# vsergeev/luaradio

Measured on NVIDIA H100. Metric: WBFM-mono chain Msamples/s (input samples) @N H100; FIR-128 HBM GB/s vs roofline, higher is better.
Workload: dtype f32

## Files before the change

### luaradio_b200/csrc/tuner.cu

```cuda
#include "common.cuh"
#include "blocks.h"

#include <cmath>
#include <cstdlib>
#include <cstring>
#include <new>
#include <string>
#include <type_traits>
#include <vector>

namespace lrb {

namespace {

#ifndef LRB_PT_THREADS
#define LRB_PT_THREADS 64
#define LRB_PT_R 8
#define LRB_PT_CTAS 8
#define LRB_PT_PREFETCH 9
#define LRB_PT_BATCH 7
#endif
#ifndef LRB_PT_CTAS_BULK
#define LRB_PT_CTAS_BULK 5
#endif
#ifndef LRB_PT_EXPERIMENT
#define LRB_PT_EXPERIMENT 0
#endif
#ifndef LRB_PT_EARLY_REST
#define LRB_PT_EARLY_REST 0
#endif
constexpr int PT_THREADS = LRB_PT_THREADS;
constexpr int PT_R = LRB_PT_R;
constexpr int PT_TO = PT_THREADS * PT_R;
constexpr int PT_MAXTAPS = 144;
constexpr int PT_BATCH = LRB_PT_BATCH;

constexpr int PT_MAXIT = 48;
struct PolyParams {
    float hr[PT_MAXTAPS];
    float hs[PT_MAXTAPS / 2];
    float2 step[PT_MAXIT];
    uint64_t turns_fix;
    uint64_t g0;
    long long off;
    int M;
    float pole_c;
    float pole_cp[6];
};
constexpr int PT_POLE_WARM = (64 % LRB_PT_R == 0) ? 64 : ((72 % LRB_PT_R == 0) ? 72 : 4 * LRB_PT_R);
static_assert(PT_POLE_WARM % LRB_PT_R == 0 && PT_POLE_WARM % 4 == 0 && PT_POLE_WARM >= 64, "pole warm-up must cover whole threads");

template <int D, int Q>
struct PolyShape {
    static constexpr int RD = PT_R * D;
    static constexpr int T = Q * D + 1;
    static constexpr int SPAN = (PT_TO + Q - 1) * D + 1;
    static constexpr int PAIRS = (SPAN + 1) / 2;
    static constexpr int ITERS = (PAIRS + PT_THREADS - 1) / PT_THREADS;
    static constexpr int LOADED = 2 * ITERS * PT_THREADS;
    __host__ __device__ static constexpr int pad(int e) { return e + 2 * (e / RD); }
    static constexpr int ELEMS = LOADED + 2 * (LOADED / RD) + 2;
    static constexpr size_t SMEM = (size_t)ELEMS * sizeof(float2);
    static constexpr int RAW = ELEMS;
    static constexpr size_t SMEM_BULK = (size_t)(ELEMS + LOADED) * sizeof(float2);
    static constexpr int NSEG = (LOADED + RD - 1) / RD;
    static constexpr int PPS = RD / 2;
    static constexpr int RG = PT_THREADS / PPS;
    static constexpr int RITERS = (NSEG + RG - 1) / RG;
};

__device__ __forceinline__ uint32_t smem_addr(const void* p) { return (uint32_t)__cvta_generic_to_shared(p); }
__device__ __forceinline__ void mbar_init(uint64_t* bar) {
    asm volatile("mbarrier.init.shared::cta.b64 [%0], 1;\n\tfence.mbarrier_init.release.cluster;\n\t"
                 "fence.proxy.async.shared::cta;" :: "r"(smem_addr(bar)) : "memory");
}
__device__ __forceinline__ void mbar_expect_tx(uint64_t* bar, uint32_t bytes) {
    asm volatile("mbarrier.arrive.expect_tx.shared::cta.b64 _, [%0], %1;" :: "r"(smem_addr(bar)), "r"(bytes) : "memory");
}
__device__ __forceinline__ void mbar_wait(uint64_t* bar, uint32_t parity) {
    asm volatile("{\n\t.reg .pred p;\n\tLRB_WAIT_%=:\n\t"
                 "mbarrier.try_wait.parity.shared::cta.b64 p, [%0], %1;\n\t"
                 "@!p bra LRB_WAIT_%=;\n\t}" :: "r"(smem_addr(bar)), "r"(parity) : "memory");
}
__device__ __forceinline__ void fence_proxy_async() { asm volatile("fence.proxy.async.shared::cta;" ::: "memory"); }
__device__ __forceinline__ void bulk_g2s(void* dst, const void* src, uint32_t bytes, uint64_t* bar) {
    asm volatile("cp.async.bulk.shared::cluster.global.mbarrier::complete_tx::bytes [%0], [%1], %2, [%3];"
                 :: "r"(smem_addr(dst)), "l"(src), "r"(bytes), "r"(smem_addr(bar)) : "memory");
}

template <int B, int E, typename F>
__device__ __forceinline__ void static_for(F&& f) {
    if constexpr (B < E) {
        f(std::integral_constant<int, B>{});
        static_for<B + 1, E>(f);
    }
}

constexpr int DISC_OV = 4;
constexpr int DISC_TAIL = 4;
template <bool DISC>
struct TileStride { static constexpr int TS = DISC ? PT_TO - DISC_OV - DISC_TAIL : PT_TO; };

template <int D, int Q, bool ROT, bool DISC, bool EDGE, bool REAL = false, bool POLE = false>
__global__ void __launch_bounds__(PT_THREADS, (!EDGE && !REAL && DISC) ? LRB_PT_CTAS_BULK : LRB_PT_CTAS)
polyphase_crcf_kernel(const float2* __restrict__ x, const float2* __restrict__ hist, long long n,
                      void* __restrict__ yv, long long n_out, const __grid_constant__ PolyParams P,
                      long long t_lo, long long t_hi,
                      const float2* __restrict__ prev_in, float2* __restrict__ prev_out, float inv_gain) {
    using S = PolyShape<D, Q>;
    static_assert(!(REAL && (ROT || DISC)), "the real-stream variant has no translator / discriminator");
    static_assert(REAL || !POLE, "the fused pole exists in the real-stream variant only");
    constexpr int PW = POLE ? PT_POLE_WARM : 0;
    constexpr int PAY = PT_TO - PW;
    constexpr int TS = REAL ? 2 * PAY : TileStride<DISC>::TS;
    constexpr int NPRE = S::ITERS < LRB_PT_PREFETCH ? S::ITERS : LRB_PT_PREFETCH;
    constexpr int LANE1 = PAY * D;
    const float* __restrict__ xr = reinterpret_cast<const float*>(x);
    const float* __restrict__ histr = reinterpret_cast<const float*>(hist);
    extern __shared__ __align__(16) float2 smem[];
    __shared__ float2 s_edge[PT_THREADS / 32];
    const int tid = threadIdx.x, lane = tid & 31, warp = tid >> 5;
    const int Hm1 = P.M - 1;

    constexpr bool BULK = !EDGE && !REAL && DISC;
    constexpr bool FFA = BULK && LRB_PT_EXPERIMENT != 2;
    __shared__ float2 s_ffa[FFA ? 4 : 1][PT_THREADS / 32];
    __shared__ __align__(8) uint64_t s_bar;
    uint32_t bar_phase = 0;

    float2 A0 = make_float2(1.f, 0.f), A1 = make_float2(1.f, 0.f);
    const int rg = tid / S::PPS, rw = tid - rg * S::PPS;
    constexpr int NE0 = (BULK && ROT) ? S::RITERS : 1;
    float2 E0[NE0];
    float2 W1 = make_float2(1.f, 0.f);
    if constexpr (BULK && ROT) {
        W1 = phasor_from_fix(P.turns_fix);
#pragma unroll
        for (int it = 0; it < NE0; ++it)
            E0[it] = phasor_from_fix(P.turns_fix * (uint64_t)((rg + S::RG * it) * S::RD + 2 * rw));
    } else if constexpr (ROT) {
        A0 = phasor_from_fix(P.turns_fix * (uint64_t)(2 * tid));
        A1 = phasor_from_fix(P.turns_fix * (uint64_t)(2 * tid + 1));
    }
    const bool rot_last = rg < S::RG && (rg + S::RG * (S::RITERS - 1)) * S::RD + 2 * rw < S::LOADED;
    auto tile_of = [&](long long idx) -> long long { return EDGE ? (idx < t_lo ? idx : t_hi + (idx - t_lo)) : (t_lo + idx); };
    const long long n_work = EDGE ? 0 : (t_hi - t_lo);
    long long widx = blockIdx.x;

    auto issue_tile = [&](long long idx) {
        if (tid == 0) {
            fence_proxy_async();
            mbar_expect_tx(&s_bar, (uint32_t)(S::LOADED * sizeof(float2)));
            bulk_g2s(smem + S::RAW, x + (P.off + tile_of(idx) * (long long)(TS * D)), (uint32_t)(S::LOADED * sizeof(float2)), &s_bar);
        }
    };
    if constexpr (BULK) {
        if (tid == 0) mbar_init(&s_bar);
        __syncthreads();
        if (widx < n_work) issue_tile(widx);
    }

    auto ld_pair = [&](long long Bt, int k) -> float4 {
        if constexpr (REAL) {
            const float2* pa = reinterpret_cast<const float2*>(xr + Bt) + (tid + k * PT_THREADS);
            const float2 a = __ldcs(pa), b = __ldcs(pa + LANE1 / 2);
            return make_float4(a.x, b.x, a.y, b.y);
        } else {
            return __ldcs(reinterpret_cast<const float4*>(x + Bt) + (tid + k * PT_THREADS));
        }
    };
    float4 pre[NPRE];
    constexpr int REST = (S::ITERS - NPRE) < PT_BATCH ? (S::ITERS - NPRE) : PT_BATCH;
    float4 rest[REST > 0 ? REST : 1];
    if constexpr (!EDGE && !BULK) {
        if (widx < n_work) {
            const long long Bt = P.off + tile_of(widx) * (long long)(TS * D);
#pragma unroll
            for (int k = 0; k < NPRE; ++k) pre[k] = ld_pair(Bt, k);
            if constexpr (LRB_PT_EARLY_REST) {
#pragma unroll
                for (int k = 0; k < REST; ++k) rest[k] = ld_pair(Bt, NPRE + k);
            }
        }
    }

    for (;;) {
        if constexpr (!EDGE) { if (widx >= n_work) break; }
        const long long tile = tile_of(widx);
        const long long B = P.off + tile * (long long)(TS * D);
        const long long m0 = tile * TS - (DISC ? DISC_OV : 0) - PW;

        auto stage_pair = [&](float4 v, int it) {
            const int u = tid + it * PT_THREADS;
            float2 a = make_float2(v.x, v.y), b = make_float2(v.z, v.w);
            if constexpr (ROT) {
                const float2 st = P.step[it];
                a = cmul(a, cmul(A0, st));
                b = cmul(b, cmul(A1, st));
            }
            *reinterpret_cast<float4*>(smem + S::pad(2 * u)) = make_float4(a.x, a.y, b.x, b.y);
        };
        if constexpr (BULK) {
            if (LRB_PT_EXPERIMENT != 1 || widx == blockIdx.x) {
                mbar_wait(&s_bar, bar_phase);
                bar_phase ^= 1;
                if (rg < S::RG) {
                    const float2* src = smem + S::RAW + rg * S::RD + 2 * rw;
                    float2* dst = smem + rg * (S::RD + 2) + 2 * rw;
#pragma unroll
                    for (int it = 0; it < S::RITERS; ++it) {
                        if (it == S::RITERS - 1 && !rot_last) break;
                        float4 v = *reinterpret_cast<const float4*>(src + it * S::RG * S::RD);
                        if constexpr (ROT) {
                            const float2 a = cmul(make_float2(v.x, v.y), E0[it]);
                            const float2 b = cmul(make_float2(v.z, v.w), cmul(E0[it], W1));
                            v = make_float4(a.x, a.y, b.x, b.y);
                        }
                        *reinterpret_cast<float4*>(dst + it * S::RG * (S::RD + 2)) = v;
                    }
                }
            }
        } else if constexpr (!EDGE && LRB_PT_EXPERIMENT == 1) {
            if (widx == blockIdx.x) {
#pragma unroll 1
                for (int it = 0; it < S::ITERS; ++it) stage_pair(ld_pair(B, it), it);
            }
        } else if constexpr (!EDGE) {
            if constexpr (!LRB_PT_EARLY_REST) {
#pragma unroll
                for (int k = 0; k < REST; ++k) rest[k] = ld_pair(B, NPRE + k);
            }
#pragma unroll
            for (int k = 0; k < NPRE; ++k) stage_pair(pre[k], k);
#pragma unroll
            for (int k = 0; k < REST; ++k) stage_pair(rest[k], NPRE + k);
#pragma unroll 1
            for (int it0 = NPRE + REST; it0 < S::ITERS; it0 += PT_BATCH) {
                float4 buf[PT_BATCH];
#pragma unroll
                for (int k = 0; k < PT_BATCH; ++k)
                    if (it0 + k < S::ITERS) buf[k] = ld_pair(B, it0 + k);
#pragma unroll
                for (int k = 0; k < PT_BATCH; ++k)
                    if (it0 + k < S::ITERS) stage_pair(buf[k], it0 + k);
            }
        } else {
#pragma unroll 7
            for (int it = 0; it < S::ITERS; ++it) {
                const long long i0 = B + 2LL * (tid + it * PT_THREADS);
                if constexpr (REAL) {
                    auto g = [&](long long i) -> float {
                        return (i >= 0) ? (i < n ? __ldg(xr + i) : 0.f) : ((Hm1 + i >= 0) ? __ldg(histr + (Hm1 + i)) : 0.f);
                    };
                    stage_pair(make_float4(g(i0), g(i0 + LANE1), g(i0 + 1), g(i0 + 1 + LANE1)), it);
                    continue;
                }
                const float2 a = (i0 >= 0) ? (i0 < n ? __ldg(x + i0) : make_float2(0.f, 0.f))
                                           : ((Hm1 + i0 >= 0) ? __ldg(hist + (Hm1 + i0)) : make_float2(0.f, 0.f));
                const long long i1 = i0 + 1;
                const float2 b = (i1 >= 0) ? (i1 < n ? __ldg(x + i1) : make_float2(0.f, 0.f))
                                           : ((Hm1 + i1 >= 0) ? __ldg(hist + (Hm1 + i1)) : make_float2(0.f, 0.f));
                stage_pair(make_float4(a.x, a.y, b.x, b.y), it);
            }
        }
        __syncthreads();

        if constexpr (BULK && LRB_PT_EXPERIMENT != 1) {
            if (widx + gridDim.x < n_work) issue_tile(widx + gridDim.x);
        }
        if constexpr (!EDGE && !BULK && LRB_PT_EXPERIMENT != 1) {
            const long long nidx = widx + gridDim.x;
            if (nidx < n_work) {
                const long long Bn = P.off + tile_of(nidx) * (long long)(TS * D);
#pragma unroll
                for (int k = 0; k < NPRE; ++k) pre[k] = ld_pair(Bn, k);
            }
        }

        float2 acc[PT_R];
#pragma unroll
        for (int r = 0; r < PT_R; ++r) acc[r] = make_float2(0.f, 0.f);
        const float2* tb = smem + tid * (S::RD + 2);
        auto load_block = [&](auto jc, float2 (&xs)[D]) {
            constexpr int j = decltype(jc)::value;
            constexpr int e0 = j * D;
            if constexpr (j == PT_R + Q - 1) {
                xs[0] = tb[S::pad(e0)];
            } else {
                static_for<0, D>([&](auto pc) {
                    constexpr int pp = decltype(pc)::value;
                    constexpr int e = e0 + pp;
                    if constexpr ((e & 1) && pp >= 1) {
                    } else if constexpr (!(e & 1) && pp + 1 < D) {
                        const float4 v = *reinterpret_cast<const float4*>(tb + S::pad(e));
                        xs[pp] = make_float2(v.x, v.y);
                        xs[pp + 1] = make_float2(v.z, v.w);
                    } else {
                        xs[pp] = tb[S::pad(e)];
                    }
                });
            }
        };
        float2 ffa_a0, ffa_fs, ffa_fb, ffa_sp;
        const float hq = P.hr[Q * D];
        if constexpr (FFA) {
            static_assert(Q % 2 == 0 && PT_R % 2 == 0 && (Q / 2) * D <= PT_MAXTAPS / 2, "fast-FIR split needs even Q and R");
            static_assert(DISC_TAIL >= 1, "the tile's last output has no A_{R/2}");
            constexpr int QH = Q / 2, KP = PT_R / 2;
            float2 fa[KP], fb[KP], fs[KP], uo[D], an;
#pragma unroll
            for (int k = 0; k < KP; ++k) fa[k] = fb[k] = fs[k] = make_float2(0.f, 0.f);
            static_for<0, PT_R + Q>([&](auto jc) {
                constexpr int j = decltype(jc)::value;
                float2 xs[D];
                load_block(jc, xs);
                if constexpr (j == PT_R + Q - 1) {
                } else if constexpr (j % 2 == 0) {
                    constexpr int i = j / 2;
                    static_for<0, KP>([&](auto kc) {
                        constexpr int k = decltype(kc)::value, q = i - k;
                        if constexpr (q >= 0 && q < QH) {
                            static_for<0, D>([&](auto pc) {
                                constexpr int pp = decltype(pc)::value;
                                const float h = P.hr[2 * q * D + pp];
                                fa[k] = ffma2(xs[pp], make_float2(h, h), fa[k]);
                            });
                        }
                    });
                    if constexpr (i >= 1 && i - 1 <= KP - 1 + QH - 1) {
                        float2 v[D];
#pragma unroll
                        for (int pp = 0; pp < D; ++pp) v[pp] = fadd2(uo[pp], xs[pp]);
                        static_for<0, KP>([&](auto kc) {
                            constexpr int k = decltype(kc)::value, q = i - 1 - k;
                            if constexpr (q >= 0 && q < QH) {
                                static_for<0, D>([&](auto pc) {
                                    constexpr int pp = decltype(pc)::value;
                                    const float h = P.hs[q * D + pp];
                                    fs[k] = ffma2(v[pp], make_float2(h, h), fs[k]);
                                });
                            }
                        });
                    }
                } else {
                    constexpr int i = (j - 1) / 2;
                    static_for<0, KP>([&](auto kc) {
                        constexpr int k = decltype(kc)::value, q = i - k;
                        if constexpr (q >= 0 && q < QH) {
                            static_for<0, D>([&](auto pc) {
                                constexpr int pp = decltype(pc)::value;
                                const float h = P.hr[(2 * q + 1) * D + pp];
                                fb[k] = ffma2(xs[pp], make_float2(h, h), fb[k]);
                            });
                        }
                    });
#pragma unroll
                    for (int pp = 0; pp < D; ++pp) uo[pp] = xs[pp];
                }
                if constexpr (j == 2 * QH - 1) {
                    an = make_float2(__shfl_down_sync(0xffffffffu, fa[0].x, 1), __shfl_down_sync(0xffffffffu, fa[0].y, 1));
                }
                if constexpr (j >= Q) {
                    constexpr int r = j - Q, k = r / 2;
                    if constexpr (r % 2 == 0) {
                        acc[r] = ffma2(xs[0], make_float2(hq, hq), fadd2(fa[k], fb[k]));
                    } else if constexpr (k + 1 < KP) {
                        acc[r] = ffma2(xs[0], make_float2(hq, hq), fsub2(fsub2(fs[k], fa[k + 1]), fb[k]));
                    } else {
                        acc[r] = ffma2(xs[0], make_float2(hq, hq), fsub2(fsub2(fs[k], an), fb[k]));
                        ffa_a0 = fa[0]; ffa_fs = fs[k]; ffa_fb = fb[k]; ffa_sp = xs[0];
                    }
                }
            });
        } else {
            static_for<0, (LRB_PT_EXPERIMENT == 2 ? 1 : PT_R + Q)>([&](auto jc) {
                constexpr int j = decltype(jc)::value;
                float2 xs[D];
                load_block(jc, xs);
                static_for<0, PT_R>([&](auto rc) {
                    constexpr int r = decltype(rc)::value;
                    constexpr int qq = j - r;
                    if constexpr (qq >= 0 && qq <= Q) {
                        static_for<0, D>([&](auto pc) {
                            constexpr int pp = decltype(pc)::value;
                            if constexpr (qq * D + pp < S::T) {
                                const float h = P.hr[qq * D + pp];
                                acc[r] = ffma2(xs[pp], make_float2(h, h), acc[r]);
                            }
                        });
                    }
                });
            });
        }
        if constexpr (!EDGE && !BULK && LRB_PT_EARLY_REST) {
            const long long nidx = widx + gridDim.x;
            if (nidx < n_work) {
                const long long Bn = P.off + tile_of(nidx) * (long long)(TS * D);
#pragma unroll
                for (int k = 0; k < REST; ++k) rest[k] = ld_pair(Bn, NPRE + k);
            }
        }
        if constexpr (ROT && !DISC) {
            const float2 Pt = phasor_from_fix(P.turns_fix * (P.g0 + (uint64_t)B));
#pragma unroll
            for (int r = 0; r < PT_R; ++r) acc[r] = cmul(acc[r], Pt);
        }

        const long long mbase = m0 + (long long)tid * PT_R;
        if constexpr (POLE) {
            const float c = P.pole_c;
            if (tile == 0 && tid < PW / PT_R) {
#pragma unroll
                for (int r = 0; r < PT_R; ++r) acc[r].x = 0.f;
                if (tid == PW / PT_R - 1) acc[PT_R - 1].x = __ldg(reinterpret_cast<const float*>(prev_in));
            }
#pragma unroll
            for (int r = 1; r < PT_R; ++r) acc[r] = ffma2(acc[r - 1], make_float2(c, c), acc[r]);
            float2 Bv = acc[PT_R - 1];
#pragma unroll
            for (int k = 0; k < 5; ++k) {
                const float2 o = make_float2(__shfl_up_sync(0xffffffffu, Bv.x, 1 << k), __shfl_up_sync(0xffffffffu, Bv.y, 1 << k));
                if (lane >= (1 << k)) Bv = ffma2(o, make_float2(P.pole_cp[k], P.pole_cp[k]), Bv);
            }
            if (lane == 31) s_edge[warp] = Bv;
            float2 prevB = make_float2(__shfl_up_sync(0xffffffffu, Bv.x, 1), __shfl_up_sync(0xffffffffu, Bv.y, 1));
            if (lane == 0) prevB = make_float2(0.f, 0.f);
            __syncthreads();
            float2 carryW = make_float2(0.f, 0.f);
            for (int w = 0; w < warp; ++w) carryW = ffma2(carryW, make_float2(P.pole_cp[5], P.pole_cp[5]), s_edge[w]);
            float f_lane = 1.f;
#pragma unroll
            for (int k = 0; k < 5; ++k) if (lane & (1 << k)) f_lane *= P.pole_cp[k];
            const float2 excl = ffma2(carryW, make_float2(f_lane, f_lane), prevB);
            float cpow = c;
#pragma unroll
            for (int r = 0; r < PT_R; ++r) { acc[r] = ffma2(excl, make_float2(cpow, cpow), acc[r]); cpow *= c; }
        }
        if constexpr (REAL) {
            float* y = reinterpret_cast<float*>(yv);
#pragma unroll
            for (int half = 0; half < 2; ++half) {
                const long long mb = mbase + half * PAY;
                if (POLE && tid < PW / PT_R) continue;
                float v[PT_R];
#pragma unroll
                for (int r = 0; r < PT_R; ++r) v[r] = half ? acc[r].y : acc[r].x;
                if (mb + PT_R <= n_out && ((reinterpret_cast<uintptr_t>(y + mb) & 15) == 0)) {
#pragma unroll
                    for (int r = 0; r < PT_R; r += 4)
                        __stcs(reinterpret_cast<float4*>(y + mb + r), make_float4(v[r], v[r + 1], v[r + 2], v[r + 3]));
                } else {
#pragma unroll
                    for (int r = 0; r < PT_R; ++r)
                        if (mb + r < n_out) y[mb + r] = v[r];
                }
                if constexpr (POLE) {
                    if (mb <= n_out - 1 && n_out - 1 < mb + PT_R) {
#pragma unroll
                        for (int r = 0; r < PT_R; ++r)
                            if (mb + r == n_out - 1) *reinterpret_cast<float*>(prev_out) = v[r];
                    }
                }
            }
            __syncthreads();
        } else if constexpr (!DISC) {
            float2* y = reinterpret_cast<float2*>(yv);
            if (mbase + PT_R <= n_out && ((reinterpret_cast<uintptr_t>(y + mbase) & 15) == 0)) {
                float4* y4 = reinterpret_cast<float4*>(y + mbase);
#pragma unroll
                for (int r = 0; r < PT_R; r += 2)
                    __stcs(y4 + r / 2, make_float4(acc[r].x, acc[r].y, acc[r + 1].x, acc[r + 1].y));
            } else {
#pragma unroll
                for (int r = 0; r < PT_R; ++r)
                    if (mbase + r < n_out) y[mbase + r] = acc[r];
            }
            __syncthreads();
        } else {
            float* yd = reinterpret_cast<float*>(yv);
            float2 left;
            left.x = __shfl_up_sync(0xffffffffu, acc[PT_R - 1].x, 1);
            left.y = __shfl_up_sync(0xffffffffu, acc[PT_R - 1].y, 1);
            if constexpr (FFA) {
                if (lane == 0) s_ffa[0][warp] = ffa_a0;
                if (lane == 31) { s_ffa[1][warp] = ffa_fs; s_ffa[2][warp] = ffa_fb; s_ffa[3][warp] = ffa_sp; }
            } else {
                if (lane == 31) s_edge[warp] = acc[PT_R - 1];
            }
            __syncthreads();
            if constexpr (FFA) {
                auto last_out = [&](int w, float2 a) {
                    return ffma2(s_ffa[3][w], make_float2(hq, hq), fsub2(fsub2(s_ffa[1][w], a), s_ffa[2][w]));
                };
                if (lane == 0 && warp > 0) left = last_out(warp - 1, ffa_a0);
                if (lane == 31 && warp + 1 < PT_THREADS / 32) acc[PT_R - 1] = last_out(warp, s_ffa[0][warp + 1]);
            } else {
                if (lane == 0 && warp > 0) left = s_edge[warp - 1];
            }
            bool zero_prev = false;
            if (EDGE && tid == 0 && tile == 0) {
                const float2 Pt = ROT ? phasor_from_fix(P.turns_fix * (P.g0 + (uint64_t)B)) : make_float2(1.f, 0.f);
                const float2 pv = __ldg(prev_in);
                acc[DISC_OV - 1] = cmul(pv, make_float2(Pt.x, -Pt.y));
                zero_prev = pv.x == 0.f && pv.y == 0.f;
            }
            const int s0 = tid * PT_R;
            float* yt = yd + m0;
            float dout[PT_R];
#pragma unroll
            for (int r = 0; r < PT_R; r += 2) {
                const float2 c0 = acc[r], p0 = (r == 0) ? left : acc[r - 1];
                const float2 c1 = acc[r + 1], p1 = acc[r];
                const float2 t0 = ffma2(c0, make_float2(p0.x, p0.x), fmul2(make_float2(c0.y, -c0.x), make_float2(p0.y, p0.y)));
                const float2 t1 = ffma2(c1, make_float2(p1.x, p1.x), fmul2(make_float2(c1.y, -c1.x), make_float2(p1.y, p1.y)));
                const float2 ang = fast_atan2f_x2(make_float2(t0.y, t1.y), make_float2(t0.x, t1.x));
                dout[r] = ang.x * inv_gain;
                dout[r + 1] = ang.y * inv_gain;
            }
            if (EDGE && zero_prev) {
                const float2 Pt = ROT ? phasor_from_fix(P.turns_fix * (P.g0 + (uint64_t)B)) : make_float2(1.f, 0.f);
                const float2 ya = ROT ? cmul(acc[DISC_OV], Pt) : acc[DISC_OV];
                const float pz = 0.f, nz = -0.f;
                const float re = __fsub_rn(__fmul_rn(ya.x, pz), __fmul_rn(ya.y, nz));
                const float im = __fadd_rn(__fmul_rn(ya.x, nz), __fmul_rn(ya.y, pz));
                dout[DISC_OV] = atan2f(im, re) * inv_gain;
            }
            if constexpr (!EDGE) {
                if (((reinterpret_cast<uintptr_t>(yt) + DISC_OV * sizeof(float)) & 15) == 0) {
                    static_assert(DISC_OV == 4 && DISC_TAIL == 4 && PT_R % 4 == 0,
                                  "thread 0 skips exactly its first float4, the last thread exactly its last");
#pragma unroll
                    for (int r = 0; r < PT_R; r += 4)
                        if ((tid > 0 || r >= DISC_OV) && (tid < PT_THREADS - 1 || r < PT_R - DISC_TAIL))
                            *reinterpret_cast<float4*>(yt + s0 + r) = make_float4(dout[r], dout[r + 1], dout[r + 2], dout[r + 3]);
                } else {
#pragma unroll
                    for (int r = 0; r < PT_R; ++r)
                        if (s0 + r >= DISC_OV && s0 + r < PT_TO - DISC_TAIL) yt[s0 + r] = dout[r];
                }
            } else {
                const long long room = n_out - m0;
                const int lim = room < (long long)(PT_TO - DISC_TAIL) ? (int)room : PT_TO - DISC_TAIL;
#pragma unroll
                for (int r = 0; r < PT_R; ++r) {
                    const int sl = s0 + r;
                    if (sl >= DISC_OV && sl < lim) {
                        yt[sl] = dout[r];
                        if ((long long)sl == room - 1) {
                            const float2 Pt = ROT ? phasor_from_fix(P.turns_fix * (P.g0 + (uint64_t)B)) : make_float2(1.f, 0.f);
                            *prev_out = cmul(acc[r], Pt);
                        }
                    }
                }
            }
        }
        if constexpr (EDGE) break;
        widx += gridDim.x;
    }
}

template <int D, int Q, bool ROT, bool DISC, bool REAL = false, bool POLE = false>
int launch_shape(PolyParams P, const float* hr_base, const float2* x, const float2* hist, long long n,
                 void* y, long long first, long long n_out, const float2* prev_in, float2* prev_out, float inv_gain,
                 cudaStream_t s) {
    using S = PolyShape<D, Q>;
    static_assert(S::T <= PT_MAXTAPS, "taps table too small");
    static bool configured_dev[LRB_MAX_DEVICES] = {false};
    static int ctas_dev[LRB_MAX_DEVICES] = {0};
    bool& configured = configured_dev[ctx().device & (LRB_MAX_DEVICES - 1)];
    int& ctas_per_sm = ctas_dev[ctx().device & (LRB_MAX_DEVICES - 1)];
    auto kern_i = polyphase_crcf_kernel<D, Q, ROT, DISC, false, REAL, POLE>;
    auto kern_e = polyphase_crcf_kernel<D, Q, ROT, DISC, true, REAL, POLE>;
    constexpr size_t SMEM_I = (!REAL && DISC) ? S::SMEM_BULK : S::SMEM;
    if (!configured) {
        LRB_CHECK(cudaFuncSetAttribute(kern_i, cudaFuncAttributeMaxDynamicSharedMemorySize, (int)SMEM_I));
        LRB_CHECK(cudaFuncSetAttribute(kern_e, cudaFuncAttributeMaxDynamicSharedMemorySize, (int)S::SMEM));
        LRB_CHECK(cudaOccupancyMaxActiveBlocksPerMultiprocessor(&ctas_per_sm, kern_i, PT_THREADS, SMEM_I));
        if (ctas_per_sm < 1) ctas_per_sm = 1;
        configured = true;
    }
    constexpr int PW = POLE ? PT_POLE_WARM : 0;
    constexpr int PAY = PT_TO - PW;
    constexpr int TS = REAL ? 2 * PAY : TileStride<DISC>::TS;
    long long off = first - (DISC ? (long long)DISC_OV * D : 0) - (long long)PW * D - (long long)(Q * D - 1);
    const int shift = (int)(((off % 2) + 2) % 2);
    off -= shift;
    P.off = off;
    for (int i = 0; i < PT_MAXTAPS; ++i) {
        const int k = i - shift;
        P.hr[i] = (k >= 0 && k < Q * D) ? hr_base[k] : 0.0f;
    }
    for (int q = 0; 2 * q + 1 < Q; ++q)
        for (int p = 0; p < D; ++p) P.hs[q * D + p] = P.hr[2 * q * D + p] + P.hr[(2 * q + 1) * D + p];
    const long long tiles = (n_out + TS - 1) / TS;
    cudaEvent_t lead_event = ctx().lead_samples > 0 ? ctx().lead_event : nullptr;
    const long long lead = lead_event ? ctx().lead_samples : 0;
    long long t_lo = 0, t_hi = 0;
    if ((reinterpret_cast<uintptr_t>(x) & (REAL ? 7 : 15)) == 0) {
        const long long step = (long long)TS * D;
        const long long need = lead - off;
        t_lo = need <= 0 ? 0 : (need + step - 1) / step;
        const long long lim = n - (long long)S::LOADED - off - (REAL ? (long long)PAY * D : 0);
        t_hi = lim < 0 ? 0 : lim / step + 1;
        if (t_hi > tiles) t_hi = tiles;
        if (DISC) {
            if (t_lo < 1) t_lo = 1;
            if (t_hi > tiles - 1) t_hi = tiles - 1;
        }
        if (t_lo > t_hi) t_lo = t_hi;
    }
    const long long n_int = t_hi - t_lo, n_edge = tiles - n_int;
    cudaStream_t side = ((n_int > 0 && n_edge > 0) || (lead_event && n_edge > 0)) ? side_fork(s) : s;
    if (n_edge > 0) {
        if (lead_event && side != s) LRB_CHECK(cudaStreamWaitEvent(side, lead_event, 0));
        else if (lead_event) LRB_CHECK(cudaStreamWaitEvent(s, lead_event, 0));
        kern_e<<<(unsigned)n_edge, PT_THREADS, S::SMEM, side>>>(x, hist, n, y, n_out, P, t_lo, t_hi, prev_in, prev_out, inv_gain);
        count_launch();
    }
    if (n_int > 0) {
        long long grid = (long long)ctx().sm_count * ctas_per_sm - ctx().reserve_ctas;
        if (grid < 1) grid = 1;
        if (grid > n_int) grid = n_int;
        kern_i<<<(unsigned)grid, PT_THREADS, SMEM_I, s>>>(x, hist, n, y, n_out, P, t_lo, t_hi, prev_in, prev_out, inv_gain);
        count_launch();
    }
    side_join(s, side);
    LRB_CHECK(cudaGetLastError());
    return 1;
}

}

struct PolyTaps {
    int M, D, Q;
    float hr[PT_MAXTAPS];
    uint64_t turns_fix;
    float2 step[PT_MAXIT];
    bool rotates = false;
    bool real_data = false;
};

static int shape_q(int M, int D, bool rotates) {
    if (D == 1 && !rotates) return M <= 16 ? 16 : (M <= 32 ? 32 : 0);
    if (D == 5 && M > 65 && M <= 128) return 26;
    return 0;
}

static int shape_q_real(int M, int D) {
    if (D == 5 && M > 130 && M <= 135) return 27;
    return 0;
}

PolyTaps* polyphase_prepare(const float* taps, int M, int D, double turns_per_sample, bool phasor_table, bool real_data) {
    int Q = real_data ? shape_q_real(M, D) : shape_q(M, D, phasor_table);
    if (!Q) return nullptr;
    PolyTaps* p = new (std::nothrow) PolyTaps();
    if (!p) return nullptr;
    p->M = M; p->D = D; p->Q = Q;
    p->real_data = real_data;
    for (int i = 0; i < PT_MAXTAPS; ++i) {
        int k = Q * D - 1 - i;
        p->hr[i] = (i < Q * D && k < M) ? taps[k] : 0.0f;
    }
    p->turns_fix = turns_to_fix(turns_per_sample);
    p->rotates = phasor_table;
    {
        const double two_pi = 6.283185307179586476925286766559;
        const long double tq = ldexpl((long double)p->turns_fix, -64);
        for (int it = 0; it < PT_MAXIT; ++it) {
            long double a = tq * (long double)(2 * PT_THREADS) * (long double)it;
            a -= floorl(a);
            p->step[it] = make_float2((float)std::cos(two_pi * (double)a), (float)std::sin(two_pi * (double)a));
        }
    }
    return p;
}

void polyphase_release(PolyTaps* p) { delete p; }

#define LRB_SHAPE_FULL(DD, QQ)                                                                                         \
    if (p->D == DD && p->Q == QQ) {                                                                                    \
        static_assert(PolyShape<DD, QQ>::ITERS <= PT_MAXIT, "step table too short");                                   \
        if (disc) return launch_shape<DD, QQ, true, true>(P, p->hr, x, hist, n, y, first, n_out, prev_in, prev_out, inv_gain, s); \
        return rot ? launch_shape<DD, QQ, true, false>(P, p->hr, x, hist, n, y, first, n_out, nullptr, nullptr, 0.f, s)    \
                   : launch_shape<DD, QQ, false, false>(P, p->hr, x, hist, n, y, first, n_out, nullptr, nullptr, 0.f, s);  \
    }
#define LRB_SHAPE_PLAIN(DD, QQ)                                                                                        \
    if (p->D == DD && p->Q == QQ && !rot && !disc) {                                                                   \
        static_assert(PolyShape<DD, QQ>::ITERS <= PT_MAXIT, "step table too short");                                   \
        return launch_shape<DD, QQ, false, false>(P, p->hr, x, hist, n, y, first, n_out, nullptr, nullptr, 0.f, s); \
    }

static int launch_polyphase_any(const PolyTaps* p, const float2* x, const float2* hist, long long n, void* y,
                                long long first, long long n_out, bool rotate, bool disc, uint64_t g0,
                                const float2* prev_in, float2* prev_out, float inv_gain, cudaStream_t s) {
    if (!p) return 0;
    if (n_out <= 0) return 1;
    const bool rot = rotate && p->rotates;
    if (disc && !rot) {
        set_error("tuner: discriminator fusion needs the translator path");
        return -1;
    }
    PolyParams P;
    std::memset(&P, 0, sizeof(P));
    P.turns_fix = p->turns_fix;
    std::memcpy(P.step, p->step, sizeof(P.step));
    P.g0 = g0;
    P.M = p->M;
    if (p->real_data) {
        if (rot || disc) { set_error("polyphase: the real-stream kernel has no translator / discriminator"); return -1; }
        const bool pole = prev_in != nullptr;
        if (pole) {
            const double c = (double)inv_gain;
            P.pole_c = inv_gain;
            double pw = std::pow(c, (double)PT_R);
            for (int k = 0; k < 6; ++k) { P.pole_cp[k] = (float)pw; pw = pw * pw; }
        }
        if (p->D == 5 && p->Q == 27)
            return pole ? launch_shape<5, 27, false, false, true, true>(P, p->hr, x, hist, n, y, first, n_out, prev_in, prev_out, 0.f, s)
                        : launch_shape<5, 27, false, false, true, false>(P, p->hr, x, hist, n, y, first, n_out, nullptr, nullptr, 0.f, s);
        return 0;
    }
    LRB_SHAPE_PLAIN(1, 16) LRB_SHAPE_PLAIN(1, 32)
    LRB_SHAPE_FULL(5, 26)
    return 0;
}

bool polyphase_pole_ok(float c) { return std::pow(std::fabs((double)c), (double)PT_POLE_WARM) <= 1e-8; }

int launch_polyphase_rrrf(const PolyTaps* p, const float* x, const float* hist, long long n, float* y,
                          long long first, long long n_out, cudaStream_t s, float pole_c, const float* z_in, float* z_out) {
    return launch_polyphase_any(p, (const float2*)x, (const float2*)hist, n, y, first, n_out, false, false, 0,
                                (const float2*)z_in, (float2*)z_out, pole_c, s);
}

int launch_polyphase_crcf(const PolyTaps* p, const float2* x, const float2* hist, long long n, float2* y,
                          long long first, long long n_out, bool rotate, uint64_t turns_fix, uint64_t g0,
                          cudaStream_t s) {
    (void)turns_fix;
    return launch_polyphase_any(p, x, hist, n, y, first, n_out, rotate, false, g0, nullptr, nullptr, 0.f, s);
}

struct TunerBlock : Block {
    int M, D;
    std::unique_ptr<PolyTaps> pt;
    DeviceBuffer d_hist[2];
    DeviceBuffer d_prev[2];
    int cur = 0, pcur = 0;
    bool disc = false;
    float gain = 1.f;
    std::string label;

    TunerBlock(std::unique_ptr<PolyTaps>&& p, float disc_gain) : M(p->M), D(p->D), pt(std::move(p)) {
        disc = disc_gain != 0.0f;
        gain = disc_gain;
        in_size = 8;
        out_size = disc ? 4 : 8;
        dev_ptrs = true;
        label = std::string(disc ? "tuner+discrim(" : "tuner(") + std::to_string(M) + ",/" + std::to_string(D) + ")";
        name = label.c_str();
    }
    int init() override {
        return carry(d_hist, (size_t)(M > 1 ? M - 1 : 1) * 8, cur) != 0 || carry(d_prev, 8, pcur) != 0 ? -1 : 0;
    }
    size_t max_output(size_t n) const override { return n / D + 1; }
    uint64_t outputs_before(uint64_t idx) const override { return (idx + D - 1) / D; }
    long long memory_in() const override { return M - 1 + (disc ? D : 0); }
    bool supports_lead_wait() const override { return true; }
    bool state_only_on_side_stream() const override { return true; }
    void rate(unsigned* up, unsigned* down) const override { *up = 1; *down = (unsigned)D; }
    int run(const void* dx, size_t n, void* dy, size_t* n_out, cudaStream_t s) override {
        long long first, no;
        decim_plan(consumed, (unsigned)D, n, &first, &no);
        *n_out = (size_t)no;
        if (n == 0) return 0;
        cudaStream_t side = s;
        if (M > 1) {
            if (n >= SIDE_STREAM_MIN) side = side_fork(s);
            if (launch_hist_update(dx, (long long)n, d_hist[cur].get(), d_hist[cur ^ 1].get(), M - 1, 8, side) != 0) return -1;
        }
        int rc = launch_polyphase_any(pt.get(), (const float2*)dx, d_hist[cur].as<const float2>(), (long long)n, dy, first, no, true,
                                      disc, consumed, d_prev[pcur].as<const float2>(), d_prev[pcur ^ 1].as<float2>(),
                                      disc ? 1.0f / gain : 0.f, s);
        side_join(s, side);
        if (rc <= 0) { if (rc == 0) set_error("tuner: unsupported shape"); return -1; }
        if (disc && no > 0) pcur ^= 1;
        if (M > 1) cur ^= 1;
        consumed += n;
        return 0;
    }
};

std::unique_ptr<Block> make_tuner(double turns_per_sample, const float* taps, int ntaps, int decim, float disc_gain) {
    std::unique_ptr<PolyTaps> p(polyphase_prepare(taps, ntaps, decim, turns_per_sample, true));
    if (!p) return nullptr;
    return make_block<TunerBlock>(std::move(p), disc_gain);
}

}
```

Baseline: 209,400.

## Stage bulk tiles via 2D TMA tensor map into padded rows in place

Replaces the flat cp.async.bulk copy into a raw staging area, followed by a padded re-copy, with a 2D TMA tensor-map load. The map uses overlapping rows (box width RD+2, row stride RD) so data lands already in the padded row layout. The rotate pass now runs in place, which removes the extra staging buffer, shrinks shared memory and drops the separate CTAS_BULK launch bound so more CTAs can be resident. The next tile's prefetch is moved later, after the post-compute sync, and new experiment switches are added. The cost is a tensor map encoded on the host every call, plus a cap on tile count from int coordinates.

```diff
diff --git a/luaradio_b200/csrc/tuner.cu b/luaradio_b200/csrc/tuner.cu
--- a/luaradio_b200/csrc/tuner.cu
+++ b/luaradio_b200/csrc/tuner.cu
@@ -1,6 +1,10 @@
 #include "common.cuh"
 #include "blocks.h"
 
+#include <cuda.h>
+#include <cudaTypedefs.h>
+
+#include <climits>
 #include <cmath>
 #include <cstdlib>
 #include <cstring>
@@ -19,9 +23,6 @@
 #define LRB_PT_CTAS 8
 #define LRB_PT_PREFETCH 9
 #define LRB_PT_BATCH 7
-#endif
-#ifndef LRB_PT_CTAS_BULK
-#define LRB_PT_CTAS_BULK 5
 #endif
 #ifndef LRB_PT_EXPERIMENT
 #define LRB_PT_EXPERIMENT 0
@@ -61,12 +62,12 @@
     __host__ __device__ static constexpr int pad(int e) { return e + 2 * (e / RD); }
     static constexpr int ELEMS = LOADED + 2 * (LOADED / RD) + 2;
     static constexpr size_t SMEM = (size_t)ELEMS * sizeof(float2);
-    static constexpr int RAW = ELEMS;
-    static constexpr size_t SMEM_BULK = (size_t)(ELEMS + LOADED) * sizeof(float2);
-    static constexpr int NSEG = (LOADED + RD - 1) / RD;
+    static constexpr int ROWS = (SPAN + RD - 1) / RD;
+    static constexpr int STAGED = ROWS * RD + 2;
+    static constexpr size_t SMEM_BULK = (size_t)ROWS * (RD + 2) * sizeof(float2);
     static constexpr int PPS = RD / 2;
     static constexpr int RG = PT_THREADS / PPS;
-    static constexpr int RITERS = (NSEG + RG - 1) / RG;
+    static constexpr int RITERS = (ROWS + RG - 1) / RG;
 };
 
 __device__ __forceinline__ uint32_t smem_addr(const void* p) { return (uint32_t)__cvta_generic_to_shared(p); }
@@ -83,9 +84,10 @@
                  "@!p bra LRB_WAIT_%=;\n\t}" :: "r"(smem_addr(bar)), "r"(parity) : "memory");
 }
 __device__ __forceinline__ void fence_proxy_async() { asm volatile("fence.proxy.async.shared::cta;" ::: "memory"); }
-__device__ __forceinline__ void bulk_g2s(void* dst, const void* src, uint32_t bytes, uint64_t* bar) {
-    asm volatile("cp.async.bulk.shared::cluster.global.mbarrier::complete_tx::bytes [%0], [%1], %2, [%3];"
-                 :: "r"(smem_addr(dst)), "l"(src), "r"(bytes), "r"(smem_addr(bar)) : "memory");
+__device__ __forceinline__ void tensor_g2s_2d(void* dst, const CUtensorMap* map, int c0, int c1, uint64_t* bar) {
+    asm volatile("cp.async.bulk.tensor.2d.shared::cluster.global.tile.mbarrier::complete_tx::bytes [%0], [%1, {%2, %3}], [%4];"
+                 :: "r"(smem_addr(dst)), "l"(reinterpret_cast<uint64_t>(map)), "r"(c0), "r"(c1), "r"(smem_addr(bar))
+                 : "memory");
 }
 
 template <int B, int E, typename F>
@@ -102,10 +104,10 @@
 struct TileStride { static constexpr int TS = DISC ? PT_TO - DISC_OV - DISC_TAIL : PT_TO; };
 
 template <int D, int Q, bool ROT, bool DISC, bool EDGE, bool REAL = false, bool POLE = false>
-__global__ void __launch_bounds__(PT_THREADS, (!EDGE && !REAL && DISC) ? LRB_PT_CTAS_BULK : LRB_PT_CTAS)
+__global__ void __launch_bounds__(PT_THREADS, LRB_PT_CTAS)
 polyphase_crcf_kernel(const float2* __restrict__ x, const float2* __restrict__ hist, long long n,
                       void* __restrict__ yv, long long n_out, const __grid_constant__ PolyParams P,
-                      long long t_lo, long long t_hi,
+                      const __grid_constant__ CUtensorMap tmap, long long t_lo, long long t_hi,
                       const float2* __restrict__ prev_in, float2* __restrict__ prev_out, float inv_gain) {
     using S = PolyShape<D, Q>;
     static_assert(!(REAL && (ROT || DISC)), "the real-stream variant has no translator / discriminator");
@@ -117,7 +119,7 @@
     constexpr int LANE1 = PAY * D;
     const float* __restrict__ xr = reinterpret_cast<const float*>(x);
     const float* __restrict__ histr = reinterpret_cast<const float*>(hist);
-    extern __shared__ __align__(16) float2 smem[];
+    extern __shared__ __align__(128) float2 smem[];
     __shared__ float2 s_edge[PT_THREADS / 32];
     const int tid = threadIdx.x, lane = tid & 31, warp = tid >> 5;
     const int Hm1 = P.M - 1;
@@ -142,16 +144,18 @@
         A0 = phasor_from_fix(P.turns_fix * (uint64_t)(2 * tid));
         A1 = phasor_from_fix(P.turns_fix * (uint64_t)(2 * tid + 1));
     }
-    const bool rot_last = rg < S::RG && (rg + S::RG * (S::RITERS - 1)) * S::RD + 2 * rw < S::LOADED;
+    const bool rot_last = rg < S::RG && rg + S::RG * (S::RITERS - 1) < S::ROWS;
     auto tile_of = [&](long long idx) -> long long { return EDGE ? (idx < t_lo ? idx : t_hi + (idx - t_lo)) : (t_lo + idx); };
     const long long n_work = EDGE ? 0 : (t_hi - t_lo);
     long long widx = blockIdx.x;
 
+    constexpr int TILE_ROWS = TS * D / S::RD;
+    static_assert(!BULK || (TS * D) % S::RD == 0, "tiles start on whole rows of the tensor map");
     auto issue_tile = [&](long long idx) {
         if (tid == 0) {
             fence_proxy_async();
-            mbar_expect_tx(&s_bar, (uint32_t)(S::LOADED * sizeof(float2)));
-            bulk_g2s(smem + S::RAW, x + (P.off + tile_of(idx) * (long long)(TS * D)), (uint32_t)(S::LOADED * sizeof(float2)), &s_bar);
+            mbar_expect_tx(&s_bar, (uint32_t)S::SMEM_BULK);
+            tensor_g2s_2d(smem, &tmap, 0, (int)(idx * TILE_ROWS), &s_bar);
         }
     };
     if constexpr (BULK) {
@@ -202,21 +206,23 @@
         };
         if constexpr (BULK) {
             if (LRB_PT_EXPERIMENT != 1 || widx == blockIdx.x) {
-                mbar_wait(&s_bar, bar_phase);
-                bar_phase ^= 1;
+                if (LRB_PT_EXPERIMENT != 3 || widx == blockIdx.x) {
+                    mbar_wait(&s_bar, bar_phase);
+                    bar_phase ^= 1;
+                }
                 if (rg < S::RG) {
-                    const float2* src = smem + S::RAW + rg * S::RD + 2 * rw;
-                    float2* dst = smem + rg * (S::RD + 2) + 2 * rw;
+                    float2* row = smem + rg * (S::RD + 2) + 2 * rw;
 #pragma unroll
                     for (int it = 0; it < S::RITERS; ++it) {
                         if (it == S::RITERS - 1 && !rot_last) break;
-                        float4 v = *reinterpret_cast<const float4*>(src + it * S::RG * S::RD);
-                        if constexpr (ROT) {
+                        float4* p = reinterpret_cast<float4*>(row + it * S::RG * (S::RD + 2));
+                        float4 v = *p;
+                        if constexpr (ROT && LRB_PT_EXPERIMENT != 4) {
                             const float2 a = cmul(make_float2(v.x, v.y), E0[it]);
                             const float2 b = cmul(make_float2(v.z, v.w), cmul(E0[it], W1));
                             v = make_float4(a.x, a.y, b.x, b.y);
                         }
-                        *reinterpret_cast<float4*>(dst + it * S::RG * (S::RD + 2)) = v;
+                        *p = v;
                     }
                 }
             }
@@ -265,9 +271,6 @@
         }
         __syncthreads();
 
-        if constexpr (BULK && LRB_PT_EXPERIMENT != 1) {
-            if (widx + gridDim.x < n_work) issue_tile(widx + gridDim.x);
-        }
         if constexpr (!EDGE && !BULK && LRB_PT_EXPERIMENT != 1) {
             const long long nidx = widx + gridDim.x;
             if (nidx < n_work) {
@@ -488,6 +491,9 @@
                 if (lane == 31) s_edge[warp] = acc[PT_R - 1];
             }
             __syncthreads();
+            if constexpr (BULK && LRB_PT_EXPERIMENT != 1 && LRB_PT_EXPERIMENT != 3) {
+                if (widx + gridDim.x < n_work) issue_tile(widx + gridDim.x);
+            }
             if constexpr (FFA) {
                 auto last_out = [&](int w, float2 a) {
                     return ffma2(s_ffa[3][w], make_float2(hq, hq), fsub2(fsub2(s_ffa[1][w], a), s_ffa[2][w]));
@@ -513,7 +519,8 @@
                 const float2 c1 = acc[r + 1], p1 = acc[r];
                 const float2 t0 = ffma2(c0, make_float2(p0.x, p0.x), fmul2(make_float2(c0.y, -c0.x), make_float2(p0.y, p0.y)));
                 const float2 t1 = ffma2(c1, make_float2(p1.x, p1.x), fmul2(make_float2(c1.y, -c1.x), make_float2(p1.y, p1.y)));
-                const float2 ang = fast_atan2f_x2(make_float2(t0.y, t1.y), make_float2(t0.x, t1.x));
+                const float2 ang = (!EDGE && LRB_PT_EXPERIMENT == 5) ? make_float2(t0.y, t1.y)
+                                                                     : fast_atan2f_x2(make_float2(t0.y, t1.y), make_float2(t0.x, t1.x));
                 dout[r] = ang.x * inv_gain;
                 dout[r + 1] = ang.y * inv_gain;
             }
@@ -557,6 +564,33 @@
         if constexpr (EDGE) break;
         widx += gridDim.x;
     }
+}
+
+int encode_tile_map(CUtensorMap* map, const float2* base, long long rows, int rd, int box_rows) {
+    static const PFN_cuTensorMapEncodeTiled encode = []() -> PFN_cuTensorMapEncodeTiled {
+        void* fn = nullptr;
+        cudaDriverEntryPointQueryResult q = cudaDriverEntryPointSymbolNotFound;
+        if (cudaGetDriverEntryPoint("cuTensorMapEncodeTiled", &fn, cudaEnableDefault, &q) != cudaSuccess ||
+            q != cudaDriverEntryPointSuccess)
+            return nullptr;
+        return reinterpret_cast<PFN_cuTensorMapEncodeTiled>(fn);
+    }();
+    if (!encode) {
+        set_error("tuner: the driver has no cuTensorMapEncodeTiled");
+        return -1;
+    }
+    const cuuint64_t dims[2] = {(cuuint64_t)(2 * (rd + 2)), (cuuint64_t)rows};
+    const cuuint64_t strides[1] = {(cuuint64_t)rd * sizeof(float2)};
+    const cuuint32_t box[2] = {(cuuint32_t)(2 * (rd + 2)), (cuuint32_t)box_rows};
+    const cuuint32_t elem_strides[2] = {1, 1};
+    const CUresult r = encode(map, CU_TENSOR_MAP_DATA_TYPE_FLOAT32, 2, const_cast<float2*>(base), dims, strides, box,
+                              elem_strides, CU_TENSOR_MAP_INTERLEAVE_NONE, CU_TENSOR_MAP_SWIZZLE_NONE,
+                              CU_TENSOR_MAP_L2_PROMOTION_L2_256B, CU_TENSOR_MAP_FLOAT_OOB_FILL_NONE);
+    if (r != CUDA_SUCCESS) {
+        set_error("tuner: cuTensorMapEncodeTiled failed (CUresult %d)", (int)r);
+        return -1;
+    }
+    return 0;
 }
 
 template <int D, int Q, bool ROT, bool DISC, bool REAL = false, bool POLE = false>
@@ -571,7 +605,10 @@
     int& ctas_per_sm = ctas_dev[ctx().device & (LRB_MAX_DEVICES - 1)];
     auto kern_i = polyphase_crcf_kernel<D, Q, ROT, DISC, false, REAL, POLE>;
     auto kern_e = polyphase_crcf_kernel<D, Q, ROT, DISC, true, REAL, POLE>;
-    constexpr size_t SMEM_I = (!REAL && DISC) ? S::SMEM_BULK : S::SMEM;
+    constexpr bool BULK = !REAL && DISC;
+    constexpr size_t SMEM_I = BULK ? S::SMEM_BULK : S::SMEM;
+    static_assert(!BULK || S::SMEM_BULK >= (size_t)(S::pad(S::SPAN - 1) + 1) * sizeof(float2),
+                  "the tensor copy covers every sample a tile reads");
     if (!configured) {
         LRB_CHECK(cudaFuncSetAttribute(kern_i, cudaFuncAttributeMaxDynamicSharedMemorySize, (int)SMEM_I));
         LRB_CHECK(cudaFuncSetAttribute(kern_e, cudaFuncAttributeMaxDynamicSharedMemorySize, (int)S::SMEM));
@@ -595,12 +632,13 @@
     const long long tiles = (n_out + TS - 1) / TS;
     cudaEvent_t lead_event = ctx().lead_samples > 0 ? ctx().lead_event : nullptr;
     const long long lead = lead_event ? ctx().lead_samples : 0;
+    const long long step = (long long)TS * D;
+    constexpr int TILE_ROWS = TS * D / S::RD;
     long long t_lo = 0, t_hi = 0;
     if ((reinterpret_cast<uintptr_t>(x) & (REAL ? 7 : 15)) == 0) {
-        const long long step = (long long)TS * D;
         const long long need = lead - off;
         t_lo = need <= 0 ? 0 : (need + step - 1) / step;
-        const long long lim = n - (long long)S::LOADED - off - (REAL ? (long long)PAY * D : 0);
+        const long long lim = n - (long long)(BULK ? S::STAGED : S::LOADED) - off - (REAL ? (long long)PAY * D : 0);
         t_hi = lim < 0 ? 0 : lim / step + 1;
         if (t_hi > tiles) t_hi = tiles;
         if (DISC) {
@@ -608,20 +646,26 @@
             if (t_hi > tiles - 1) t_hi = tiles - 1;
         }
         if (t_lo > t_hi) t_lo = t_hi;
+        if (BULK && t_hi - t_lo > (INT_MAX - S::ROWS) / TILE_ROWS) t_hi = t_lo + (INT_MAX - S::ROWS) / TILE_ROWS;
     }
     const long long n_int = t_hi - t_lo, n_edge = tiles - n_int;
+    CUtensorMap tmap;
+    std::memset(&tmap, 0, sizeof(tmap));
+    if (BULK && n_int > 0 &&
+        encode_tile_map(&tmap, x + off + t_lo * step, (n_int - 1) * TILE_ROWS + S::ROWS, S::RD, S::ROWS) != 0)
+        return -1;
     cudaStream_t side = ((n_int > 0 && n_edge > 0) || (lead_event && n_edge > 0)) ? side_fork(s) : s;
     if (n_edge > 0) {
         if (lead_event && side != s) LRB_CHECK(cudaStreamWaitEvent(side, lead_event, 0));
         else if (lead_event) LRB_CHECK(cudaStreamWaitEvent(s, lead_event, 0));
-        kern_e<<<(unsigned)n_edge, PT_THREADS, S::SMEM, side>>>(x, hist, n, y, n_out, P, t_lo, t_hi, prev_in, prev_out, inv_gain);
+        kern_e<<<(unsigned)n_edge, PT_THREADS, S::SMEM, side>>>(x, hist, n, y, n_out, P, tmap, t_lo, t_hi, prev_in, prev_out, inv_gain);
         count_launch();
     }
     if (n_int > 0) {
         long long grid = (long long)ctx().sm_count * ctas_per_sm - ctx().reserve_ctas;
         if (grid < 1) grid = 1;
         if (grid > n_int) grid = n_int;
-        kern_i<<<(unsigned)grid, PT_THREADS, SMEM_I, s>>>(x, hist, n, y, n_out, P, t_lo, t_hi, prev_in, prev_out, inv_gain);
+        kern_i<<<(unsigned)grid, PT_THREADS, SMEM_I, s>>>(x, hist, n, y, n_out, P, tmap, t_lo, t_hi, prev_in, prev_out, inv_gain);
         count_launch();
     }
     side_join(s, side);
```

New measurement: 223,200 (median of 6 runs). 1.07x the previous value.
